# edielsonpf/speech-recognition-hmm-continuous

Measured on NVIDIA B200. Metric: frames/sec per Baum-Welch EM iteration, higher is better.
Workload: dtype f32

## Files before the change

### speech_recognition_hmm_continuous_b200/csrc/acch_kernels.cuh

```cuda
#pragma once

#include <cuda_fp16.h>

#include "dec_kernels.cuh"
#include "ws_kernels.cuh"

namespace hmmk {

constexpr int kAhSub = 64;
constexpr int kAhStages = 4;
constexpr int kAhDrain = 8;
constexpr int kAhCfWarps = kAhSub / 32;
constexpr int kAhProdWarp = 8 + kAhCfWarps;
constexpr int kAhG1Warp = kAhProdWarp + 1;
constexpr int kAhThreads = (kAhG1Warp + 2) * 32;
constexpr int kAhTmS = 256, kAhTmW = 352;
constexpr float kAhWLog2 = 14.f;

__host__ __device__ inline size_t ah_tile_bytes(int KP) { return (size_t)2 * (kAhSub / 8) * (3 * KP / 16) * 128; }
__host__ __device__ inline size_t ah_image_bytes(int KP) { return (size_t)128 * 2 * KP * 2; }
__host__ __device__ inline size_t ah_stage_bytes(int KP) { return ah_tile_bytes(KP) + kAhSub * 8 * 4; }
__host__ __device__ inline size_t ah_smem_bytes(int KP) { return kAhStages * ah_stage_bytes(KP) + 1024 + 256 + kAccImgCap * 4 + (size_t)KP * 128 * 4; }

constexpr int kAhScN = 7;
// ... 33 lines not shown
      const float *src = x32 + (int64_t)__ldg(frame_ids + tl.x + f) * DP + cc * 8;
      const float *s = sc + blk * DP + cc * 8;
      const float4 a = __ldg(reinterpret_cast<const float4 *>(src)), b = __ldg(reinterpret_cast<const float4 *>(src + 4));
      float v[8] = {a.x, a.y, a.z, a.w, b.x, b.y, b.z, b.w};
#pragma unroll
      for (int j = 0; j < 8; j++) v[j] = (blk != 1 ? v[j] * v[j] : v[j]) * s[j];
      split_half2(v[0], v[1], h.x, l.x); split_half2(v[2], v[3], h.y, l.y);
      split_half2(v[4], v[5], h.z, l.z); split_half2(v[6], v[7], h.w, l.w);
    }
    const size_t o = (size_t)fg * NCH * 128 + (size_t)c * 128 + (size_t)r * 16;
    *reinterpret_cast<uint4 *>(hi + o) = h;
    *reinterpret_cast<uint4 *>(lo + o) = l;
  }
}

__global__ void k_pack_wT_h(const double *__restrict__ mu, const double *__restrict__ iv, const float *__restrict__ kc2all,
                            const double *__restrict__ ctr, const float *__restrict__ sc, int G, int nRB, int D, int DP,
                            unsigned short *__restrict__ images, float *__restrict__ kcT) {
  const int img = blockIdx.y, v = img / nRB, rb = img - v * nRB;
  const int KP = 2 * DP;
  pdl_wait();
  unsigned short *im = images + (size_t)img * (ah_image_bytes(KP) / 2);
  for (int idx = blockIdx.x * blockDim.x + threadIdx.x; idx < 128 * KP; idx += gridDim.x * blockDim.x) {
    const int r = idx / KP, k = idx - r * KP;
    const int part = k / DP, d = k - part * DP;
    const int g = rb * 128 + r;
    float val = 0.f;
    if (g < G && d < D) {
      const int64_t gg = (int64_t)v * G + g;
      const double m = mu[gg * D + d] - ctr[d], w = iv[gg * D + d];
      val = (float)(part == 1 ? m * w * (double)sc[4 * DP + d] : -0.5 * w * (double)sc[3 * DP + d]);
    }
    unsigned short h, l;
    split_half(val, h, l);
    im[(size_t)r * 2 * KP + k] = h;
    im[(size_t)r * 2 * KP + KP + k] = l;
    if (k == 0) kcT[(size_t)img * 128 + r] = (g < G) ? kc2all[(int64_t)v * G + g] : kNegInf;
  }
}

__device__ __forceinline__ void bulk_copy_g2s(uint32_t dst_smem, const void *src, uint32_t bytes, uint32_t mbar) {
  asm volatile("cp.async.bulk.shared::cluster.global.mbarrier::complete_tx::bytes [%0], [%1], %2, [%3];" ::"r"(dst_smem), "l"(src), "r"(bytes),
               "r"(mbar)
               : "memory");
}

__global__ void __launch_bounds__(kAhThreads, 1)
k_accum_h(const TcTile *__restrict__ units, int nunits, const int32_t *__restrict__ frame_ids, const unsigned char *__restrict__ x16,
          const uint32_t *__restrict__ images, const float *__restrict__ kcT, const float *__restrict__ logb, const float *__restrict__ gamma,
          int N, int M, int G, int D, int DP, double *__restrict__ stats, int64_t stats_stride, int64_t off_S0, int64_t off_S1, int64_t off_S2,
          float *__restrict__ scratch, const float *__restrict__ dsc) {
// ... 292 lines not shown
```

### speech_recognition_hmm_continuous_b200/csrc/hmmcu.cu

```cuda
#include <cuda_runtime.h>
#include <stdarg.h>
#include <stdio.h>
#include <string.h>

#include <algorithm>
#include <atomic>
#include <map>
#include <string>
#include <utility>
#include <vector>

#include "hmm_cuda.h"
#include "kernels.cuh"
#include "fb_kernels.cuh"
#include "fbres_kernels.cuh"
#include "tc_kernels.cuh"
#include "ws_kernels.cuh"
#include "dec_kernels.cuh"
#include "acch_kernels.cuh"
#include "vit_kernels.cuh"
#include "init_kernels.cuh"

using namespace hmmk;

namespace {

char g_create_err[512] = "";
std::atomic<uint64_t> g_alloc_epoch{0};

struct DevBuf {
  void *p = nullptr;
  size_t cap = 0;
  cudaError_t ensure(size_t bytes) {
    if (bytes <= cap) return cudaSuccess;
    g_alloc_epoch++;
    if (p) cudaFree(p);
// ... 58 lines not shown
  int use_graph = 1;
  uint64_t cfg_epoch = 0;
  GraphSlot g_estep, g_mstep;
  int train_path = 0;
  std::map<std::string, Timer> timers;

  int U = 0, D = 0, DP = 0, Tmax = 0;
  int64_t F = 0;
  bool have_features = false;
  DevBuf x64_own;
  const double *d_x64 = nullptr;
  DevBuf x32, ctr, off_d, xabs_d;
  std::vector<int64_t> off;
  double kappa = 0.0;
  bool kappa_stale = true;
  DevBuf em_old, em_active, ctl_d, ext_d, upd_d;
  double *ctl_h = nullptr;
  size_t ctl_cap = 0;

  int V = 0, N = 0, M = 0, G = 0, Dm = 0;
  bool have_models = false, pack_dirty = true;
  bool banded = false;
  DevBuf A, c, mu, iv, det, mu32, iv32, k32, kc2;
  bool kc_dirty = true, simt_dirty = true;

  std::vector<int32_t> u2m;
  DevBuf u2m_d, mus_d, mu_d, tiles_d;
  DevBuf vit_map, vit_tiles;
  std::vector<int32_t> vit_u2m;
  int64_t n_vit_tiles = 0;
  uint64_t feat_epoch = 1, vit_epoch = 0;
// ... 237 lines not shown
}

void hmmcu_destroy(hmmcu_ctx *ctx) {
  if (!ctx) return;
  cudaSetDevice(ctx->dev);
  cudaStreamSynchronize(ctx->st);
  unlink_streams(ctx);
  for (void *p : ctx->peer_opened) cudaIpcCloseMemHandle(p);
  ctx->peer_area.release(); ctx->peer_ptrs_d.release(); ctx->peer_seq_d.release(); ctx->peer_stamps.release();
  ctx->logb_joint.release();
  DevBuf *bufs[] = {&ctx->x64_own, &ctx->x32, &ctx->ctr, &ctx->off_d, &ctx->A, &ctx->c, &ctx->mu, &ctx->iv, &ctx->det,
                    &ctx->mu32, &ctx->iv32, &ctx->k32, &ctx->kc2, &ctx->u2m_d, &ctx->mus_d, &ctx->mu_d, &ctx->tiles_d, &ctx->logb,
                    &ctx->post, &ctx->gamma, &ctx->alpha_ws, &ctx->stats, &ctx->logp_utt_d, &ctx->score_d,
                    &ctx->psi_ws, &ctx->path_d, &ctx->tiles_dec, &ctx->rank_in, &ctx->rank_out, &ctx->tc_train.images, &ctx->tc_train.kc, &ctx->tc_train.s0,
                    &ctx->tc_train.ns, &ctx->xabs_d, &ctx->tc_dec.images, &ctx->tc_dec.kc, &ctx->tc_dec.s0, &ctx->tc_dec.ns, &ctx->tc_tiles_train,
                    &ctx->frame_ids_d, &ctx->tc_tiles_dec, &ctx->acc_images, &ctx->acc_kc, &ctx->acc_units, &ctx->beta_ws, &ctx->acc_dbg, &ctx->em_old, &ctx->em_active, &ctx->ctl_d, &ctx->ext_d, &ctx->upd_d, &ctx->ws_train.images, &ctx->ws_train.s0, &ctx->ws_train.ns,
                    &ctx->ws_dec.images, &ctx->ws_dec.images16, &ctx->ws_dec.scales16, &ctx->ws_dec.s0, &ctx->ws_dec.ns, &ctx->ws_tiles_train, &ctx->acc_units64, &ctx->logb64, &ctx->acc_scratch, &ctx->acc_slot_start, &ctx->acc_slot_ids, &ctx->in_lst, &ctx->in_off, &ctx->in_vk, &ctx->in_cent,
                    &ctx->in_sum, &ctx->in_dist, &ctx->in_cnt, &ctx->in_idx, &ctx->in_dd, &ctx->in_ord, &ctx->vit_map, &ctx->vit_tiles,
                    &ctx->res_order, &ctx->res_upos, &ctx->res_batches, &ctx->res_counter, &ctx->ustats,
                    &ctx->acc_images16, &ctx->acc_sc, &ctx->acc_unitsH, &ctx->acc_slot_start_h, &ctx->acc_slot_ids_h, &ctx->x16, &ctx->x16_tiles};
  for (DevBuf *b : bufs) b->release();
  for (auto &kv : ctx->timers) {
    if (kv.second.a) cudaEventDestroy(kv.second.a);
    if (kv.second.b) cudaEventDestroy(kv.second.b);
    for (auto &pr : kv.second.pairs) { cudaEventDestroy(pr.first); cudaEventDestroy(pr.second); }
  }
  if (ctx->g_estep.exec) cudaGraphExecDestroy(ctx->g_estep.exec);
  if (ctx->g_mstep.exec) cudaGraphExecDestroy(ctx->g_mstep.exec);
  if (ctx->ctl_h) cudaFreeHost(ctx->ctl_h);
  if (ctx->ctr_h) cudaFreeHost(ctx->ctr_h);
  if (ctx->path_h) cudaFreeHost(ctx->path_h);
// ... 18 lines not shown
  CK(cudaSetDevice(ctx->dev));
  CK(cudaStreamSynchronize(ctx->st));
  return HMMCU_OK;
}
int hmmcu_host_alloc(void **p, uint64_t bytes) { return cudaMallocHost(p, bytes) == cudaSuccess ? HMMCU_OK : HMMCU_ENOMEM; }
void hmmcu_host_free(void *p) {
  if (p) cudaFreeHost(p);
}
int64_t hmmcu_launch_count(const hmmcu_ctx *ctx) { return ctx ? ctx->launches : 0; }
void hmmcu_enable_timing(hmmcu_ctx *ctx, int on) { ctx->timing = on != 0; ctx->cfg_epoch++; }
double hmmcu_last_kernel_ms(const hmmcu_ctx *ctx, const char *name) {
  if (strcmp(name, "kappa") == 0) return ctx->kappa;
  if (strcmp(name, "tc_active") == 0) return ctx->last_tc ? 1.0 : 0.0;
  if (strcmp(name, "dec_f16_active") == 0) return ctx->last_dec16 ? 1.0 : 0.0;
  if (strcmp(name, "acc_h_active") == 0) return ctx->last_acc_h ? 1.0 : 0.0;
  if (strcmp(name, "dec_grid") == 0) return (double)ctx->dec_grid;
  {
    const size_t ln = strlen(name);
    if (ln > 6 && strcmp(name + ln - 6, "_total") == 0) {
      auto itt = ctx->timers.find(std::string(name, ln - 6));
      if (itt == ctx->timers.end() || !itt->second.used) return -1.0;
      const Timer &t = itt->second;
      if (!t.collect) return hmmcu_last_kernel_ms(ctx, std::string(name, ln - 6).c_str());
      double tot = 0.0;
      for (size_t k = 0; k < t.npairs; k++) {
        float ms1 = 0.f;
        if (cudaEventSynchronize(t.pairs[k].second) != cudaSuccess || cudaEventElapsedTime(&ms1, t.pairs[k].first, t.pairs[k].second) != cudaSuccess) {
          cudaGetLastError();
          return -1.0;
        }
// ... 1601 lines not shown
  std::vector<int> act(V, 1);
  CK(cudaMemcpyAsync(ctx->em_old.p, one.data(), sizeof(double) * V, cudaMemcpyHostToDevice, ctx->st));
  CK(cudaMemcpyAsync(ctx->em_active.p, act.data(), sizeof(int) * V, cudaMemcpyHostToDevice, ctx->st));
  CK(cudaStreamSynchronize(ctx->st));
  return HMMCU_OK;
}

int hmmcu_mstep(hmmcu_ctx *ctx, double threshold, double *sum_logp, double *n_utt, int32_t *updated) {
  if (!ctx || !ctx->have_models || ctx->stats_n != hmmcu_stats_size(ctx->N, ctx->M, ctx->Dm) * ctx->V || !ctx->em_old.p)
    return fail(ctx, HMMCU_EINVAL, "mstep: needs hmmcu_em_reset and an E-step on the current model set");
  CK(cudaSetDevice(ctx->dev));
  const int V = ctx->V;
  int rc = ensure_ctl(ctx);
  if (rc) return rc;
  const int64_t ssz = hmmcu_stats_size(ctx->N, ctx->M, ctx->Dm);
  CK(ctx->upd_d.ensure(sizeof(int) * V));
  {
    const int DP = round_up(ctx->Dm + 1, 4);
    CK(ctx->ext_d.ensure(sizeof(unsigned long long) * (2 * DP + 1)));
  }
  const bool repack = ctx->train_path == 2 && !ctx->pack_dirty && !ctx->ws_train.dirty && !ctx->acc_dirty && !ctx->kc_dirty &&
                      ctx->have_features && ctx->Dm == ctx->D;
  auto enqueue = [&]() -> int {
    t_begin(ctx, "mstep");
    k_mstep_ctl<<<(V + 127) / 128, 128, 0, ctx->st>>>(ctx->stats.as<double>(), ssz, V, threshold, ctx->em_old.as<double>(),
                                                      ctx->em_active.as<int>(), ctx->ctl_d.as<double>(), ctx->upd_d.as<int>());
    LAUNCH_CHECK();
    CK(launch_pdl(k_mstep_apply, dim3(1 + (ctx->G + 7) / 8, V), 256, 0, ctx->st, ctx->stats.as<double>(), ssz, ctx->N, ctx->M, ctx->Dm,
                  1.0e-5 , ctx->upd_d.as<int>(), ctx->A.as<double>(), ctx->c.as<double>(),
                  ctx->mu.as<double>(), ctx->iv.as<double>(), ctx->det.as<double>()));
    LAUNCH_CHECK();
    int rc2;
    const bool fork = !ctx->timing && ctx->mstep_fork;
    auto on_stream = [&](cudaStream_t side, auto launch) -> int {
      cudaStream_t keep = ctx->st;
      ctx->st = side;
      const int r = launch();
      ctx->st = keep;
      return r;
    };
    if (fork) {
      CK(cudaEventRecord(ctx->ev_fork[0], ctx->st));
      CK(cudaStreamWaitEvent(ctx->st_aux[0], ctx->ev_fork[0], 0));
      if ((rc2 = on_stream(ctx->st_aux[0], [&] { return launch_kappa(ctx, ctx->ctl_d.as<double>() + 3 * V); })) != HMMCU_OK) return rc2;
      CK(cudaEventRecord(ctx->ev_join[0], ctx->st_aux[0]));
    } else {
      if ((rc2 = launch_kappa(ctx, ctx->ctl_d.as<double>() + 3 * V)) != HMMCU_OK) return rc2;
    }
    t_end(ctx, "mstep");
    if (repack) {
      t_begin(ctx, "pack");
      if ((rc2 = launch_pack_kc(ctx)) != HMMCU_OK) return rc2;
      if (fork) {
        CK(cudaEventRecord(ctx->ev_fork[1], ctx->st));
        CK(cudaStreamWaitEvent(ctx->st_aux[1], ctx->ev_fork[1], 0));
        if ((rc2 = on_stream(ctx->st_aux[1], [&] { return launch_pack_acc(ctx); })) != HMMCU_OK) return rc2;
        CK(cudaEventRecord(ctx->ev_join[1], ctx->st_aux[1]));
      }
      if ((rc2 = launch_pack_ws(ctx, ctx->ws_train)) != HMMCU_OK) return rc2;
      if (fork) CK(cudaStreamWaitEvent(ctx->st, ctx->ev_join[1], 0));
      else if ((rc2 = launch_pack_acc(ctx)) != HMMCU_OK) return rc2;
      t_end(ctx, "pack");
    }
    if (fork) CK(cudaStreamWaitEvent(ctx->st, ctx->ev_join[0], 0));
    CK(cudaMemcpyAsync(ctx->ctl_h, ctx->ctl_d.p, sizeof(double) * (3 * (size_t)V + 1), cudaMemcpyDeviceToHost, ctx->st));
    return HMMCU_OK;
  };
  uint64_t tbits;
  memcpy(&tbits, &threshold, sizeof(tbits));
  if ((rc = run_graphed(ctx, ctx->g_mstep, (tbits * 31u) ^ (repack ? 2u : 0u) ^ (ctx->mstep_fork ? 4u : 0u), enqueue)) != HMMCU_OK) return rc;
  CK(cudaStreamSynchronize(ctx->st));
  for (int v = 0; v < V; v++) {
    if (sum_logp) sum_logp[v] = ctx->ctl_h[v];
    if (n_utt) n_utt[v] = ctx->ctl_h[V + v];
    if (updated) updated[v] = ctx->ctl_h[2 * V + v] != 0.0;
  }
  ctx->kappa = ctx->ctl_h[3 * V];
  ctx->kappa_stale = false;
  if (repack) {
    ctx->simt_dirty = true;
    ctx->tc_train.dirty = true;
    ctx->tc_dec.dirty = true;
    ctx->ws_dec.dirty = true;
  } else {
    ctx->pack_dirty = true;
// ... 494 lines not shown
```

### speech_recognition_hmm_continuous_b200/csrc/kernels.cuh

```cuda
#pragma once
#include <cuda_runtime.h>
#include <math.h>
#include <stdint.h>

namespace hmmk {

constexpr float kNegInf = -INFINITY;
constexpr double kLogTrueMin = -744.4400719213812;

__host__ __device__ inline int round_up(int a, int b) { return (a + b - 1) / b * b; }

__device__ __forceinline__ void pdl_wait() { asm volatile("griddepcontrol.wait;" ::: "memory"); }
__device__ __forceinline__ void pdl_trigger() { asm volatile("griddepcontrol.launch_dependents;" ::: "memory"); }

__global__ void k_center(const double *__restrict__ x, int64_t F, int D, int DP, double *__restrict__ ctr) {
  __shared__ double part[16][64];
  const int d = threadIdx.x & 63, grp = threadIdx.x >> 6;
  int64_t ns = F < 4096 ? F : 4096;
  int64_t stride = F / ns;
  for (int d0 = 0; d0 < DP; d0 += 64) {
    double s = 0.0;
    if (d0 + d < D)
      for (int64_t k = grp; k < ns; k += 16) s += x[(k * stride) * D + d0 + d];
    part[grp][d] = s;
// ... 340 lines not shown
    else if (e0 < 2) sec = 1;
    else {
      int b2 = -1;
      for (int k = 0; k < e0; k++) {
        if (k == best) continue;
        if (b2 < 0 || val(k) > val(b2)) b2 = k;
      }
      sec = b2;
    }
  }
  label[u] = first;
  if (second) second[u] = sec;
}


__global__ void k_mstep_ctl(const double *__restrict__ stats, int64_t ss, int V, double threshold, double *__restrict__ em_old,
                            int *__restrict__ em_active, double *__restrict__ ctl, int *__restrict__ upd) {
  const int v = blockIdx.x * blockDim.x + threadIdx.x;
  pdl_trigger();
  if (v >= V) return;
  const double *st = stats + (int64_t)v * ss;
  const double probab = st[ss - 2], nutt = st[ss - 1];
  ctl[v] = probab;
  ctl[V + v] = nutt;
  int u = 0;
  if (em_active[v]) {
    const double variation = fabs((em_old[v] - probab) / em_old[v]);
    if (variation > threshold) { em_old[v] = probab; u = 1; }
    else em_active[v] = 0;
  }
  ctl[2 * V + v] = (double)u;
  upd[v] = u;
}

__global__ void __launch_bounds__(256)
k_mstep_apply(const double *__restrict__ stats, int64_t ss, int N, int M, int D, double floor_, const int *__restrict__ upd,
              double *__restrict__ Aall, double *__restrict__ call, double *__restrict__ muall, double *__restrict__ ivall,
              double *__restrict__ detall) {
  const int v = blockIdx.y, tid = threadIdx.x, G = N * M;
  pdl_wait();
  pdl_trigger();
  if (!upd[v]) return;
  const double *st = stats + (int64_t)v * ss;
  const double *num = st, *den = num + (int64_t)N * N, *denmix = den + N, *S0 = denmix + N;
  const double *S1 = S0 + G, *S2 = S1 + (int64_t)G * D;
  if (blockIdx.x == 0) {
    double *A = Aall + (int64_t)v * N * N, *c = call + (int64_t)v * G;
    for (int idx = tid; idx < N * N; idx += blockDim.x) {
      const int i = idx / N;
      if (den[i] != 0.0) A[idx] = num[idx] / den[i];
    }
    for (int i = tid; i < N; i += blockDim.x) {
      double *w = c + i * M;
      if (denmix[i] != 0.0)
        for (int k = 0; k < M; k++) w[k] = S0[i * M + k] / denmix[i];
      double s = 0.0;
      for (int k = 0; k < M; k++) {
        if (w[k] < floor_) w[k] = floor_;
        s += w[k];
      }
      for (int k = 0; k < M; k++) w[k] /= s;
    }
    return;
  }
  const int warp = tid >> 5, lane = tid & 31;
  const int k = (blockIdx.x - 1) * 8 + warp;
  if (k >= G) return;
  const int i = k / M;
  double *mu = muall + ((int64_t)v * G + k) * D, *iv = ivall + ((int64_t)v * G + k) * D;
  const bool fresh = denmix[i] != 0.0;
  const double s0 = S0[k];
  double dt = 1.0;
  for (int d0 = 0; d0 < D; d0 += 32) {
    const int d = d0 + lane;
    double var = 1.0;
    if (d < D) {
      if (fresh) {
        mu[d] = S1[(int64_t)k * D + d] / s0;
        var = S2[(int64_t)k * D + d] / s0;
        if (var < floor_) var = floor_;
      } else var = iv[d];
      iv[d] = 1.0 / var;
    }
    const int nd = min(32, D - d0);
    for (int j = 0; j < nd; j++) dt *= __shfl_sync(0xffffffffu, var, j);
  }
  if (lane == 0) detall[(int64_t)v * G + k] = dt;
}

__global__ void k_model_extremes(const double *__restrict__ mu, const double *__restrict__ iv, const double *__restrict__ ctr,
                                 int64_t VG, int D, int DP, unsigned long long *__restrict__ ext, const unsigned int *__restrict__ xabs,
                                 unsigned int *__restrict__ done, double *__restrict__ kappa_out) {
  const int d = threadIdx.x % DP, grp = threadIdx.x / DP, ngrp = blockDim.x / DP;
  if (d < D && grp < ngrp) {
    double ivm = 0.0, mum = 0.0;
    const double c0 = ctr[d];
    for (int64_t g = (int64_t)blockIdx.x * ngrp + grp; g < VG; g += (int64_t)gridDim.x * ngrp) {
      double a = iv[g * D + d], b = fabs(mu[g * D + d] - c0);
      if (!(a == a)) a = INFINITY;
      if (!(b == b)) b = INFINITY;
      ivm = fmax(ivm, a);
      mum = fmax(mum, b);
    }
    atomicMax(ext + d, (unsigned long long)__double_as_longlong(ivm));
    atomicMax(ext + DP + d, (unsigned long long)__double_as_longlong(mum));
  }
  __shared__ bool last;
  __threadfence();
  __syncthreads();
  if (threadIdx.x == 0) last = atomicAdd(done, 1u) == gridDim.x - 1;
  __syncthreads();
  if (!last) return;
  __threadfence();
  __shared__ double part[8];
  double t = 0.0;
  for (int dd = threadIdx.x; dd < D; dd += blockDim.x) {
    const double ivm = __longlong_as_double((long long)__ldcg(ext + dd));
    double r = __longlong_as_double((long long)__ldcg(ext + DP + dd));
    if (xabs) r = fmax(r, (double)__uint_as_float(xabs[dd]));
    const double u = 2.0 * ivm * r * r;
    t += (u == u) ? u : INFINITY;
  }
#pragma unroll
  for (int o = 16; o > 0; o >>= 1) t += __shfl_xor_sync(0xffffffffu, t, o);
  if ((threadIdx.x & 31) == 0 && (threadIdx.x >> 5) < 8) part[threadIdx.x >> 5] = t;
  __syncthreads();
  if (threadIdx.x == 0) {
    double kappa = 0.0;
    for (int w = 0; w < min(8, (int)(blockDim.x + 31) / 32); w++) kappa += part[w];
    *kappa_out = kappa;
  }
}

}
```

### speech_recognition_hmm_continuous_b200/csrc/tc_kernels.cuh

```cuda
#pragma once
#include <cuda_runtime.h>
#include <stdint.h>

#include "kernels.cuh"

namespace hmmk {

constexpr int kTcRows = 128;
constexpr int kTcThreads = 256;
constexpr int kTcMaxTN = 192;

struct TcTile {
  int32_t row0;
  int32_t nrows;
  int32_t img;
  int32_t state0;
  int32_t v;
  int32_t pad;
};

__host__ __device__ inline int tc_slab_bytes(int rows) { return rows * 32; }
__host__ __device__ inline size_t tc_image_bytes(int TN, int KP) { return (size_t)2 * (KP / 8) * tc_slab_bytes(TN); }
__host__ __device__ inline uint32_t tc_elem_off(int row, int k) {
  return (uint32_t)((row >> 3) * 256 + (((k & 7) >> 2) * 128) + ((row & 7) * 16) + ((k & 3) * 4));
// ... 330 lines not shown
__device__ __forceinline__ void tmem_wait_ld() { asm volatile("tcgen05.wait::ld.sync.aligned;" ::: "memory"); }
__device__ __forceinline__ void tmem_st16(uint32_t taddr, const uint32_t *r) {
  asm volatile(
      "tcgen05.st.sync.aligned.32x32b.x16.b32 [%0], {%1,%2,%3,%4,%5,%6,%7,%8,%9,%10,%11,%12,%13,%14,%15,%16};" ::"r"(taddr),
      "r"(r[0]), "r"(r[1]), "r"(r[2]), "r"(r[3]), "r"(r[4]), "r"(r[5]), "r"(r[6]), "r"(r[7]), "r"(r[8]), "r"(r[9]), "r"(r[10]),
      "r"(r[11]), "r"(r[12]), "r"(r[13]), "r"(r[14]), "r"(r[15])
      : "memory");
}
__device__ __forceinline__ void tmem_st8(uint32_t taddr, const uint32_t *r) {
  asm volatile("tcgen05.st.sync.aligned.32x32b.x8.b32 [%0], {%1,%2,%3,%4,%5,%6,%7,%8};" ::"r"(taddr), "r"(r[0]), "r"(r[1]), "r"(r[2]),
               "r"(r[3]), "r"(r[4]), "r"(r[5]), "r"(r[6]), "r"(r[7])
               : "memory");
}
__device__ __forceinline__ void tmem_wait_st() { asm volatile("tcgen05.wait::st.sync.aligned;" ::: "memory"); }

__global__ void k_pack_kc(const double *__restrict__ mu, const double *__restrict__ iv, const double *__restrict__ det,
                          const double *__restrict__ c, const double *__restrict__ ctr, int64_t VG, int D, float *__restrict__ kc2) {
  const int64_t g = ((int64_t)blockIdx.x * blockDim.x + threadIdx.x) >> 5;
  const int lane = threadIdx.x & 31;
  pdl_wait();
  pdl_trigger();
  if (g >= VG) return;
  double q = 0.0;
  for (int d = lane; d < D; d += 32) {
    const double m = mu[g * D + d] - ctr[d];
    q += m * m * iv[g * D + d];
  }
#pragma unroll
  for (int o = 16; o > 0; o >>= 1) q += __shfl_xor_sync(0xffffffffu, q, o);
  if (lane == 0) {
    double k = -INFINITY;
    const double dt = det[g], cc = c[g];
    if (dt != 0.0 && cc > 0.0) k = (log(cc) - 0.5 * ((double)D * 1.8378770664093453 + log(fabs(dt))) - 0.5 * q) * 1.4426950408889634;
    kc2[g] = (float)k;
  }
}

__global__ void k_pack_wT_tc(const double *__restrict__ mu, const double *__restrict__ iv, const float *__restrict__ kc2all,
                             const double *__restrict__ ctr, int G, int nRB, int D, int DP, float *__restrict__ images,
                             float *__restrict__ kcT) {
  const int img = blockIdx.y, v = img / nRB, rb = img - v * nRB;
  const int KP = 2 * DP;
  float *im = images + (size_t)img * (tc_accT_image_bytes(KP) / 4);
  for (int idx = blockIdx.x * blockDim.x + threadIdx.x; idx < 128 * KP; idx += gridDim.x * blockDim.x) {
    const int r = idx / KP, k = idx - r * KP;
    const int part = k / DP, d = k - part * DP;
    const int g = rb * 128 + r;
    float val = 0.f;
    if (g < G && d < D) {
      const int64_t gg = (int64_t)v * G + g;
      const double m = mu[gg * D + d] - ctr[d], w = iv[gg * D + d];
      val = (float)(part == 0 ? m * w : -0.5 * w);
    }
    float h, l;
    split_tf32(val, h, l);
    im[(size_t)r * 2 * KP + k] = h;
    im[(size_t)r * 2 * KP + KP + k] = l;
    if (k == 0) kcT[(size_t)img * 128 + r] = (g < G) ? kc2all[(int64_t)v * G + g] : kNegInf;
  }
}

__global__ void __launch_bounds__(kTcThreads, 1)
k_accum_tc(const TcTile *__restrict__ units, int nunits, const int32_t *__restrict__ frame_ids, const float *__restrict__ x32,
           const float *__restrict__ images, const float *__restrict__ kcT, const float *__restrict__ logb,
           const float *__restrict__ gamma, int N, int M, int G, int D, int DP, double *__restrict__ stats,
           int64_t stats_stride, int64_t off_S0, int64_t off_S1, int64_t off_S2, float *__restrict__ dbg) {
  extern __shared__ __align__(1024) uint8_t smem_raw[];
  __shared__ uint64_t mbar;
  __shared__ uint32_t tmem_base_s;
  const int KP = 2 * DP, KP2 = tc_kp2(KP), NSLAB = KP / 8;
  const uint32_t PX = (uint32_t)(KP / 4) * 128;
  uint8_t *sm = (uint8_t *)(((uintptr_t)smem_raw + 1023) & ~(uintptr_t)1023);
// ... 227 lines not shown
```

### speech_recognition_hmm_continuous_b200/csrc/ws_kernels.cuh

```cuda
#pragma once
#include <cuda_fp16.h>
#include "tc_kernels.cuh"

namespace hmmk {

constexpr int kWsEpiWarps = 8;
constexpr int kWsThreads = (kWsEpiWarps + 9) * 32;
constexpr int kWsMaxTN = 96;
constexpr int kWsMaxTN1 = 176;
constexpr int kWsXch = 6;

__host__ __device__ inline size_t ws_image_bytes(int TN, int KP) { return (size_t)2 * (TN / 8) * (KP / 4) * 128 + (size_t)TN * 4; }
__host__ __device__ inline size_t ws_emis_smem_bytes(int TN, int KP) { return ws_image_bytes(TN, KP) + 1024 + 272; }

__host__ __device__ inline int ws_pad_m(int M) {
  if (M > 16) return (M + 15) / 16 * 16;
  if (M == 3 || M == 5) return M;
  int p = 1;
  while (p < M) p <<= 1;
  return p;
}
__host__ __device__ inline int ws_states_per_chunk(int MPd) { return MPd <= 16 ? 16 / MPd : 1; }
__host__ __device__ inline int ws_image_cols(int MPd, int nstates) {
  if (MPd > 16) return nstates * MPd;
// ... 57 lines not shown
  float4 v;
  asm volatile("ld.shared.v4.f32 {%0, %1, %2, %3}, [%4];" : "=f"(v.x), "=f"(v.y), "=f"(v.z), "=f"(v.w) : "r"(addr));
  return v;
}
__device__ __forceinline__ float lds_f32(uint32_t addr) {
  float v;
  asm volatile("ld.shared.f32 %0, [%1];" : "=f"(v) : "r"(addr));
  return v;
}
__device__ __forceinline__ int lds_i32(uint32_t addr) {
  int v;
  asm volatile("ld.shared.s32 %0, [%1];" : "=r"(v) : "r"(addr));
  return v;
}
__device__ __forceinline__ void sts_f32(uint32_t addr, float v) { asm volatile("st.shared.f32 [%0], %1;" ::"r"(addr), "f"(v) : "memory"); }

__global__ void k_pack_w_ws(const double *__restrict__ mu, const double *__restrict__ iv, const float *__restrict__ kc2all,
                            const double *__restrict__ ctr, int M, int MP, int D, int DP, int TN,
                            const int32_t *__restrict__ img_state0, const int32_t *__restrict__ img_nstates,
                            float *__restrict__ images) {
  const int img = blockIdx.y;
  const int KP = 2 * DP;
  pdl_wait();
  const uint32_t P = (uint32_t)(KP / 4) * 128;
  const size_t img_floats = ws_image_bytes(TN, KP) / 4;
  float *hi = images + (size_t)img * img_floats;
  float *lo = hi + (size_t)(TN / 8) * (P / 4);
  float *kc2 = lo + (size_t)(TN / 8) * (P / 4);
  const int64_t s0g = img_state0[img];
  const int nst = img_nstates[img];
  auto gauss_of = [&](int n) -> int64_t {
    int st, m;
    if (MP > 16) { st = n / MP; m = n - st * MP; }
    else {
      const int spc = 16 / MP, c = n >> 4, w = n & 15;
      if (w >= spc * MP) return -1;
      st = c * spc + w / MP; m = w % MP;
    }
    return (st < nst && m < M) ? (s0g + st) * M + m : -1;
  };
  for (int idx = blockIdx.x * blockDim.x + threadIdx.x; idx < TN * KP; idx += gridDim.x * blockDim.x) {
    const int n = idx / KP, k = idx - n * KP;
    const int part = k / DP, d = k - part * DP;
    const int64_t g = gauss_of(n);
    float val = 0.f;
    if (g >= 0 && d < D) {
      const double m = mu[g * D + d] - ctr[d], w = iv[g * D + d];
      val = (float)(part == 0 ? m * w : -0.5 * w);
    }
    float h, l;
    split_tf32(val, h, l);
    const size_t o = ((size_t)(n & 7) * 16 + (k & 3) * 4 + (size_t)(k >> 2) * 128 + (size_t)(n >> 3) * P) / 4;
    hi[o] = h;
    lo[o] = l;
    if (k == 0) kc2[n] = (g >= 0) ? kc2all[g] : kNegInf;
  }
}

__host__ __device__ inline size_t dec16_image_bytes(int TN, int KP) { return (size_t)2 * (TN / 8) * (KP / 8) * 128 + (size_t)TN * 4; }

__global__ void k_dec16_scales(const unsigned long long *__restrict__ ext, const unsigned int *__restrict__ xabs, int D, int DP, float *__restrict__ sc) {
  const int d = threadIdx.x;
  if (d >= DP) return;
  float s1 = 1.f, s2 = 1.f;
  bool dead = false;
  if (d < D) {
    const double ivm = __longlong_as_double((long long)ext[d]), mum = __longlong_as_double((long long)ext[DP + d]);
    const double r = xabs ? (double)__uint_as_float(xabs[d]) : mum;
    const double wl = mum * ivm;
// ... 903 lines not shown
```

Baseline: 1.801 billion.

## Fuse M-step control, update, kappa, and weight repacking into one kernel

Replaces the M-step pipeline with a single kernel launched one CTA per (state, model). The old pipeline was a control kernel, an apply kernel, a kappa/extremes kernel on a forked stream and three pack kernels. The new kernel updates A, mixture weights, means, variances and determinants, and writes the tensor-core weight images and kc2 constants in place. A last-block reduction then computes the per-dimension extremes, kappa and the control flags. This removes several launches, a stream fork and join, and re-reading mu/iv for packing. In exchange it relies on a grid-wide last-block pattern with atomics and a persistent scratch buffer, and it drops the device-to-host copy of the control array, which is now written directly to a host pointer.

Result: faster. 1.978 billion (median of 6 runs) (+9.8%).

```diff
diff --git a/speech_recognition_hmm_continuous_b200/csrc/acch_kernels.cuh b/speech_recognition_hmm_continuous_b200/csrc/acch_kernels.cuh
--- a/speech_recognition_hmm_continuous_b200/csrc/acch_kernels.cuh
+++ b/speech_recognition_hmm_continuous_b200/csrc/acch_kernels.cuh
@@ -71,6 +71,16 @@
   }
 }
 
+__device__ __forceinline__ float w_h_val(double mu, double iv, double ctr, const float *sc, int DP, int d, int part) {
+  const double m = mu - ctr;
+  return (float)(part == 1 ? m * iv * (double)sc[4 * DP + d] : -0.5 * iv * (double)sc[3 * DP + d]);
+}
+__device__ __forceinline__ void acc_h_put(unsigned short *im, int KP, int r, int k, float val) {
+  unsigned short h, l;
+  split_half(val, h, l);
+  im[(size_t)r * 2 * KP + k] = h;
+  im[(size_t)r * 2 * KP + KP + k] = l;
+}
 __global__ void k_pack_wT_h(const double *__restrict__ mu, const double *__restrict__ iv, const float *__restrict__ kc2all,
                             const double *__restrict__ ctr, const float *__restrict__ sc, int G, int nRB, int D, int DP,
                             unsigned short *__restrict__ images, float *__restrict__ kcT) {
@@ -85,13 +95,9 @@
     float val = 0.f;
     if (g < G && d < D) {
       const int64_t gg = (int64_t)v * G + g;
-      const double m = mu[gg * D + d] - ctr[d], w = iv[gg * D + d];
-      val = (float)(part == 1 ? m * w * (double)sc[4 * DP + d] : -0.5 * w * (double)sc[3 * DP + d]);
-    }
-    unsigned short h, l;
-    split_half(val, h, l);
-    im[(size_t)r * 2 * KP + k] = h;
-    im[(size_t)r * 2 * KP + KP + k] = l;
+      val = w_h_val(mu[gg * D + d], iv[gg * D + d], ctr[d], sc, DP, d, part);
+    }
+    acc_h_put(im, KP, r, k, val);
     if (k == 0) kcT[(size_t)img * 128 + r] = (g < G) ? kc2all[(int64_t)v * G + g] : kNegInf;
   }
 }
diff --git a/speech_recognition_hmm_continuous_b200/csrc/hmmcu.cu b/speech_recognition_hmm_continuous_b200/csrc/hmmcu.cu
--- a/speech_recognition_hmm_continuous_b200/csrc/hmmcu.cu
+++ b/speech_recognition_hmm_continuous_b200/csrc/hmmcu.cu
@@ -20,6 +20,7 @@
 #include "acch_kernels.cuh"
 #include "vit_kernels.cuh"
 #include "init_kernels.cuh"
+#include "mstep_kernels.cuh"
 
 using namespace hmmk;
 
@@ -108,7 +109,8 @@
   std::vector<int64_t> off;
   double kappa = 0.0;
   bool kappa_stale = true;
-  DevBuf em_old, em_active, ctl_d, ext_d, upd_d;
+  DevBuf em_old, em_active, ctl_d, ext_d;
+  DevBuf mstep_scr;
   double *ctl_h = nullptr;
   size_t ctl_cap = 0;
 
@@ -376,7 +378,7 @@
                     &ctx->post, &ctx->gamma, &ctx->alpha_ws, &ctx->stats, &ctx->logp_utt_d, &ctx->score_d,
                     &ctx->psi_ws, &ctx->path_d, &ctx->tiles_dec, &ctx->rank_in, &ctx->rank_out, &ctx->tc_train.images, &ctx->tc_train.kc, &ctx->tc_train.s0,
                     &ctx->tc_train.ns, &ctx->xabs_d, &ctx->tc_dec.images, &ctx->tc_dec.kc, &ctx->tc_dec.s0, &ctx->tc_dec.ns, &ctx->tc_tiles_train,
-                    &ctx->frame_ids_d, &ctx->tc_tiles_dec, &ctx->acc_images, &ctx->acc_kc, &ctx->acc_units, &ctx->beta_ws, &ctx->acc_dbg, &ctx->em_old, &ctx->em_active, &ctx->ctl_d, &ctx->ext_d, &ctx->upd_d, &ctx->ws_train.images, &ctx->ws_train.s0, &ctx->ws_train.ns,
+                    &ctx->frame_ids_d, &ctx->tc_tiles_dec, &ctx->acc_images, &ctx->acc_kc, &ctx->acc_units, &ctx->beta_ws, &ctx->acc_dbg, &ctx->em_old, &ctx->em_active, &ctx->ctl_d, &ctx->ext_d, &ctx->mstep_scr, &ctx->ws_train.images, &ctx->ws_train.s0, &ctx->ws_train.ns,
                     &ctx->ws_dec.images, &ctx->ws_dec.images16, &ctx->ws_dec.scales16, &ctx->ws_dec.s0, &ctx->ws_dec.ns, &ctx->ws_tiles_train, &ctx->acc_units64, &ctx->logb64, &ctx->acc_scratch, &ctx->acc_slot_start, &ctx->acc_slot_ids, &ctx->in_lst, &ctx->in_off, &ctx->in_vk, &ctx->in_cent,
                     &ctx->in_sum, &ctx->in_dist, &ctx->in_cnt, &ctx->in_idx, &ctx->in_dd, &ctx->in_ord, &ctx->vit_map, &ctx->vit_tiles,
                     &ctx->res_order, &ctx->res_upos, &ctx->res_batches, &ctx->res_counter, &ctx->ustats,
@@ -425,6 +427,7 @@
   if (strcmp(name, "tc_active") == 0) return ctx->last_tc ? 1.0 : 0.0;
   if (strcmp(name, "dec_f16_active") == 0) return ctx->last_dec16 ? 1.0 : 0.0;
   if (strcmp(name, "acc_h_active") == 0) return ctx->last_acc_h ? 1.0 : 0.0;
+  if (strcmp(name, "train_path") == 0) return (double)ctx->train_path;
   if (strcmp(name, "dec_grid") == 0) return (double)ctx->dec_grid;
   {
     const size_t ln = strlen(name);
@@ -2056,61 +2059,52 @@
   int rc = ensure_ctl(ctx);
   if (rc) return rc;
   const int64_t ssz = hmmcu_stats_size(ctx->N, ctx->M, ctx->Dm);
-  CK(ctx->upd_d.ensure(sizeof(int) * V));
+  const int N = ctx->N, M = ctx->M, D = ctx->Dm, DP = round_up(D + 1, 4);
+  CK(ctx->ext_d.ensure(sizeof(unsigned long long) * (2 * DP + 1)));
   {
-    const int DP = round_up(ctx->Dm + 1, 4);
-    CK(ctx->ext_d.ensure(sizeof(unsigned long long) * (2 * DP + 1)));
+    const size_t cap0 = ctx->mstep_scr.cap;
+    CK(ctx->mstep_scr.ensure(sizeof(unsigned long long) * (2 * DP + 1)));
+    if (ctx->mstep_scr.cap != cap0) CK(cudaMemsetAsync(ctx->mstep_scr.p, 0, ctx->mstep_scr.cap, ctx->st));
   }
   const bool repack = ctx->train_path == 2 && !ctx->pack_dirty && !ctx->ws_train.dirty && !ctx->acc_dirty && !ctx->kc_dirty &&
                       ctx->have_features && ctx->Dm == ctx->D;
+  MstepPack pk = {};
+  if (repack) {
+    hmmcu_ctx::TcSet &ts = ctx->ws_train;
+    pk.kc2 = ctx->kc2.as<float>();
+    pk.ws = ts.images.as<float>();
+    pk.ws_TN = ts.TN;
+    pk.ws_SCt = ts.SCt;
+    pk.ws_ipw = (N + ts.SCt - 1) / ts.SCt;
+    pk.ws_MP = ws_pad_m(M);
+    if (h_acc_on(ctx)) {
+      pk.acc_h = ctx->acc_images16.as<unsigned short>();
+      pk.acc_sc = ctx->acc_sc.as<float>();
+    } else {
+      pk.acc_tc = ctx->acc_images.as<float>();
+    }
+    pk.acc_kc = ctx->acc_kc.as<float>();
+    pk.nRB = (ctx->G + 127) / 128;
+  }
+  const int threads = 32 * std::min(std::max(M, 8), 16);
+  const size_t smem = sizeof(double) * (M + 2 * (size_t)DP);
+  if (smem > 227 * 1024) return fail(ctx, HMMCU_EINVAL, "mstep: M=%d, D=%d do not fit one CTA's shared memory", M, D);
+  if (smem > 48 * 1024) CK(cudaFuncSetAttribute(k_mstep, cudaFuncAttributeMaxDynamicSharedMemorySize, (int)smem));
   auto enqueue = [&]() -> int {
     t_begin(ctx, "mstep");
-    k_mstep_ctl<<<(V + 127) / 128, 128, 0, ctx->st>>>(ctx->stats.as<double>(), ssz, V, threshold, ctx->em_old.as<double>(),
-                                                      ctx->em_active.as<int>(), ctx->ctl_d.as<double>(), ctx->upd_d.as<int>());
+    k_mstep<<<dim3(N, V), threads, smem, ctx->st>>>(ctx->stats.as<double>(), ssz, V, N, M, D, DP, 1.0e-5 ,
+                                                     threshold, ctx->em_old.as<double>(), ctx->em_active.as<int>(), ctx->A.as<double>(),
+                                                     ctx->c.as<double>(), ctx->mu.as<double>(), ctx->iv.as<double>(), ctx->det.as<double>(),
+                                                     ctx->ctr.as<double>(), pk, ctx->mstep_scr.as<unsigned long long>(),
+                                                     ctx->ext_d.as<unsigned long long>(), ctx->F > 0 ? ctx->xabs_d.as<unsigned int>() : nullptr,
+                                                     ctx->ctl_h);
     LAUNCH_CHECK();
-    CK(launch_pdl(k_mstep_apply, dim3(1 + (ctx->G + 7) / 8, V), 256, 0, ctx->st, ctx->stats.as<double>(), ssz, ctx->N, ctx->M, ctx->Dm,
-                  1.0e-5 , ctx->upd_d.as<int>(), ctx->A.as<double>(), ctx->c.as<double>(),
-                  ctx->mu.as<double>(), ctx->iv.as<double>(), ctx->det.as<double>()));
-    LAUNCH_CHECK();
-    int rc2;
-    const bool fork = !ctx->timing && ctx->mstep_fork;
-    auto on_stream = [&](cudaStream_t side, auto launch) -> int {
-      cudaStream_t keep = ctx->st;
-      ctx->st = side;
-      const int r = launch();
-      ctx->st = keep;
-      return r;
-    };
-    if (fork) {
-      CK(cudaEventRecord(ctx->ev_fork[0], ctx->st));
-      CK(cudaStreamWaitEvent(ctx->st_aux[0], ctx->ev_fork[0], 0));
-      if ((rc2 = on_stream(ctx->st_aux[0], [&] { return launch_kappa(ctx, ctx->ctl_d.as<double>() + 3 * V); })) != HMMCU_OK) return rc2;
-      CK(cudaEventRecord(ctx->ev_join[0], ctx->st_aux[0]));
-    } else {
-      if ((rc2 = launch_kappa(ctx, ctx->ctl_d.as<double>() + 3 * V)) != HMMCU_OK) return rc2;
-    }
     t_end(ctx, "mstep");
-    if (repack) {
-      t_begin(ctx, "pack");
-      if ((rc2 = launch_pack_kc(ctx)) != HMMCU_OK) return rc2;
-      if (fork) {
-        CK(cudaEventRecord(ctx->ev_fork[1], ctx->st));
-        CK(cudaStreamWaitEvent(ctx->st_aux[1], ctx->ev_fork[1], 0));
-        if ((rc2 = on_stream(ctx->st_aux[1], [&] { return launch_pack_acc(ctx); })) != HMMCU_OK) return rc2;
-        CK(cudaEventRecord(ctx->ev_join[1], ctx->st_aux[1]));
-      }
-      if ((rc2 = launch_pack_ws(ctx, ctx->ws_train)) != HMMCU_OK) return rc2;
-      if (fork) CK(cudaStreamWaitEvent(ctx->st, ctx->ev_join[1], 0));
-      else if ((rc2 = launch_pack_acc(ctx)) != HMMCU_OK) return rc2;
-      t_end(ctx, "pack");
-    }
-    if (fork) CK(cudaStreamWaitEvent(ctx->st, ctx->ev_join[0], 0));
-    CK(cudaMemcpyAsync(ctx->ctl_h, ctx->ctl_d.p, sizeof(double) * (3 * (size_t)V + 1), cudaMemcpyDeviceToHost, ctx->st));
     return HMMCU_OK;
   };
   uint64_t tbits;
   memcpy(&tbits, &threshold, sizeof(tbits));
-  if ((rc = run_graphed(ctx, ctx->g_mstep, (tbits * 31u) ^ (repack ? 2u : 0u) ^ (ctx->mstep_fork ? 4u : 0u), enqueue)) != HMMCU_OK) return rc;
+  if ((rc = run_graphed(ctx, ctx->g_mstep, (tbits * 31u) ^ (repack ? 2u : 0u), enqueue)) != HMMCU_OK) return rc;
   CK(cudaStreamSynchronize(ctx->st));
   for (int v = 0; v < V; v++) {
     if (sum_logp) sum_logp[v] = ctx->ctl_h[v];
diff --git a/speech_recognition_hmm_continuous_b200/csrc/kernels.cuh b/speech_recognition_hmm_continuous_b200/csrc/kernels.cuh
--- a/speech_recognition_hmm_continuous_b200/csrc/kernels.cuh
+++ b/speech_recognition_hmm_continuous_b200/csrc/kernels.cuh
@@ -378,78 +378,28 @@
 }
 
 
-__global__ void k_mstep_ctl(const double *__restrict__ stats, int64_t ss, int V, double threshold, double *__restrict__ em_old,
-                            int *__restrict__ em_active, double *__restrict__ ctl, int *__restrict__ upd) {
-  const int v = blockIdx.x * blockDim.x + threadIdx.x;
-  pdl_trigger();
-  if (v >= V) return;
-  const double *st = stats + (int64_t)v * ss;
-  const double probab = st[ss - 2], nutt = st[ss - 1];
-  ctl[v] = probab;
-  ctl[V + v] = nutt;
-  int u = 0;
-  if (em_active[v]) {
-    const double variation = fabs((em_old[v] - probab) / em_old[v]);
-    if (variation > threshold) { em_old[v] = probab; u = 1; }
-    else em_active[v] = 0;
-  }
-  ctl[2 * V + v] = (double)u;
-  upd[v] = u;
-}
-
-__global__ void __launch_bounds__(256)
-k_mstep_apply(const double *__restrict__ stats, int64_t ss, int N, int M, int D, double floor_, const int *__restrict__ upd,
-              double *__restrict__ Aall, double *__restrict__ call, double *__restrict__ muall, double *__restrict__ ivall,
-              double *__restrict__ detall) {
-  const int v = blockIdx.y, tid = threadIdx.x, G = N * M;
-  pdl_wait();
-  pdl_trigger();
-  if (!upd[v]) return;
-  const double *st = stats + (int64_t)v * ss;
-  const double *num = st, *den = num + (int64_t)N * N, *denmix = den + N, *S0 = denmix + N;
-  const double *S1 = S0 + G, *S2 = S1 + (int64_t)G * D;
-  if (blockIdx.x == 0) {
-    double *A = Aall + (int64_t)v * N * N, *c = call + (int64_t)v * G;
-    for (int idx = tid; idx < N * N; idx += blockDim.x) {
-      const int i = idx / N;
-      if (den[i] != 0.0) A[idx] = num[idx] / den[i];
-    }
-    for (int i = tid; i < N; i += blockDim.x) {
-      double *w = c + i * M;
-      if (denmix[i] != 0.0)
-        for (int k = 0; k < M; k++) w[k] = S0[i * M + k] / denmix[i];
-      double s = 0.0;
-      for (int k = 0; k < M; k++) {
-        if (w[k] < floor_) w[k] = floor_;
-        s += w[k];
-      }
-      for (int k = 0; k < M; k++) w[k] /= s;
-    }
-    return;
-  }
-  const int warp = tid >> 5, lane = tid & 31;
-  const int k = (blockIdx.x - 1) * 8 + warp;
-  if (k >= G) return;
-  const int i = k / M;
-  double *mu = muall + ((int64_t)v * G + k) * D, *iv = ivall + ((int64_t)v * G + k) * D;
-  const bool fresh = denmix[i] != 0.0;
-  const double s0 = S0[k];
-  double dt = 1.0;
-  for (int d0 = 0; d0 < D; d0 += 32) {
-    const int d = d0 + lane;
-    double var = 1.0;
-    if (d < D) {
-      if (fresh) {
-        mu[d] = S1[(int64_t)k * D + d] / s0;
-        var = S2[(int64_t)k * D + d] / s0;
-        if (var < floor_) var = floor_;
-      } else var = iv[d];
-      iv[d] = 1.0 / var;
-    }
-    const int nd = min(32, D - d0);
-    for (int j = 0; j < nd; j++) dt *= __shfl_sync(0xffffffffu, var, j);
-  }
-  if (lane == 0) detall[(int64_t)v * G + k] = dt;
+__device__ __forceinline__ void extremes_kappa(const unsigned long long *ext, const unsigned int *xabs, int D, int DP, double *kappa_out) {
+  __shared__ double part[8];
+  const int tid = threadIdx.x;
+  if (tid < 256) {
+    double t = 0.0;
+    for (int dd = tid; dd < D; dd += 256) {
+      const double ivm = __longlong_as_double((long long)__ldcg(ext + dd));
+      double r = __longlong_as_double((long long)__ldcg(ext + DP + dd));
+      if (xabs) r = fmax(r, (double)__uint_as_float(xabs[dd]));
+      const double u = 2.0 * ivm * r * r;
+      t += (u == u) ? u : INFINITY;
+    }
+#pragma unroll
+    for (int o = 16; o > 0; o >>= 1) t += __shfl_xor_sync(0xffffffffu, t, o);
+    if ((tid & 31) == 0) part[tid >> 5] = t;
+  }
+  __syncthreads();
+  if (tid == 0) {
+    double kappa = 0.0;
+    for (int w = 0; w < 8; w++) kappa += part[w];
+    *kappa_out = kappa;
+  }
 }
 
 __global__ void k_model_extremes(const double *__restrict__ mu, const double *__restrict__ iv, const double *__restrict__ ctr,
@@ -476,24 +426,7 @@
   __syncthreads();
   if (!last) return;
   __threadfence();
-  __shared__ double part[8];
-  double t = 0.0;
-  for (int dd = threadIdx.x; dd < D; dd += blockDim.x) {
-    const double ivm = __longlong_as_double((long long)__ldcg(ext + dd));
-    double r = __longlong_as_double((long long)__ldcg(ext + DP + dd));
-    if (xabs) r = fmax(r, (double)__uint_as_float(xabs[dd]));
-    const double u = 2.0 * ivm * r * r;
-    t += (u == u) ? u : INFINITY;
-  }
-#pragma unroll
-  for (int o = 16; o > 0; o >>= 1) t += __shfl_xor_sync(0xffffffffu, t, o);
-  if ((threadIdx.x & 31) == 0 && (threadIdx.x >> 5) < 8) part[threadIdx.x >> 5] = t;
-  __syncthreads();
-  if (threadIdx.x == 0) {
-    double kappa = 0.0;
-    for (int w = 0; w < min(8, (int)(blockDim.x + 31) / 32); w++) kappa += part[w];
-    *kappa_out = kappa;
-  }
-}
-
-}
+  extremes_kappa(ext, xabs, D, DP, kappa_out);
+}
+
+}
diff --git a/speech_recognition_hmm_continuous_b200/csrc/mstep_kernels.cuh b/speech_recognition_hmm_continuous_b200/csrc/mstep_kernels.cuh
--- /dev/null
+++ b/speech_recognition_hmm_continuous_b200/csrc/mstep_kernels.cuh
@@ -0,0 +1,186 @@
+#pragma once
+
+#include "acch_kernels.cuh"
+
+namespace hmmk {
+
+__device__ __forceinline__ int mstep_rule(double probab, double old, int active, double threshold) {
+  if (!active) return 0;
+  const double variation = fabs((old - probab) / old);
+  return variation > threshold ? 1 : 0;
+}
+
+struct MstepPack {
+  float *kc2;
+  float *ws;
+  int ws_TN, ws_SCt, ws_ipw, ws_MP;
+  float *acc_tc;
+  unsigned short *acc_h;
+  const float *acc_sc;
+  float *acc_kc;
+  int nRB;
+};
+
+__global__ void __launch_bounds__(512)
+k_mstep(const double *__restrict__ stats, int64_t ss, int V, int N, int M, int D, int DP, double floor_, double threshold,
+        double *__restrict__ em_old, int *__restrict__ em_active, double *__restrict__ Aall, double *__restrict__ call,
+        double *__restrict__ muall, double *__restrict__ ivall, double *__restrict__ detall, const double *__restrict__ ctr,
+        MstepPack pk, unsigned long long *__restrict__ scr, unsigned long long *__restrict__ ext,
+        const unsigned int *__restrict__ xabs, double *__restrict__ ctl) {
+  extern __shared__ double sm_w[];
+  unsigned long long *sx = reinterpret_cast<unsigned long long *>(sm_w + M);
+  __shared__ double s_sum;
+  __shared__ bool last;
+  const int i = blockIdx.x, v = blockIdx.y, tid = threadIdx.x, warp = tid >> 5, lane = tid & 31, nw = blockDim.x >> 5;
+  const int G = N * M, KP = 2 * DP;
+  for (int t = tid; t < 2 * DP; t += blockDim.x) sx[t] = 0ull;
+
+  const double *st = stats + (int64_t)v * ss;
+  const int u = mstep_rule(st[ss - 2], em_old[v], em_active[v], threshold);
+  const double *num = st, *den = num + (int64_t)N * N, *denmix = den + N, *S0 = denmix + N;
+  const double *S1 = S0 + G, *S2 = S1 + (int64_t)G * D;
+  const bool fresh = u && denmix[i] != 0.0;
+
+  double *cst = call + (int64_t)v * G + (int64_t)i * M;
+  if (u) {
+    if (den[i] != 0.0)
+      for (int j = tid; j < N; j += blockDim.x) Aall[(int64_t)v * N * N + i * N + j] = num[i * N + j] / den[i];
+    for (int m = tid; m < M; m += blockDim.x) {
+      double w = fresh ? S0[i * M + m] / denmix[i] : cst[m];
+      if (w < floor_) w = floor_;
+      sm_w[m] = w;
+    }
+  }
+  __syncthreads();
+  if (u && tid == 0) {
+    double s = 0.0;
+    for (int m = 0; m < M; m++) s += sm_w[m];
+    s_sum = s;
+  }
+  __syncthreads();
+  if (u)
+    for (int m = tid; m < M; m += blockDim.x) {
+      const double w = sm_w[m] / s_sum;
+      sm_w[m] = w;
+      cst[m] = w;
+    }
+  __syncthreads();
+
+  const bool pack = u && pk.ws != nullptr;
+  const uint32_t P = (uint32_t)(KP / 4) * 128;
+  float *ws_hi = nullptr, *ws_lo = nullptr, *ws_kc = nullptr;
+  double ivm0 = 0.0, mum0 = 0.0, ivm1 = 0.0, mum1 = 0.0;
+  if (pack) {
+    ws_hi = pk.ws + (size_t)(v * pk.ws_ipw + i / pk.ws_SCt) * (ws_image_bytes(pk.ws_TN, KP) / 4);
+    ws_lo = ws_hi + (size_t)(pk.ws_TN / 8) * (P / 4);
+    ws_kc = ws_lo + (size_t)(pk.ws_TN / 8) * (P / 4);
+  }
+  for (int m = warp; m < M; m += nw) {
+    const int gi = i * M + m;
+    const int64_t g = (int64_t)v * G + gi;
+    double *mu = muall + g * D, *iv = ivall + g * D;
+    const double s0 = fresh ? S0[gi] : 1.0;
+    const int n = pack ? ws_row_of(i % pk.ws_SCt, m, pk.ws_MP) : 0;
+    const int aimg = v * pk.nRB + gi / 128, ar = gi % 128;
+    double dt = 1.0, q = 0.0;
+    for (int d0 = 0; d0 < D; d0 += 32) {
+      const int d = d0 + lane;
+      double var = 1.0;
+      if (d < D) {
+        double mud, ivd;
+        const double cd = ctr[d];
+        if (u) {
+          if (fresh) {
+            mud = S1[(int64_t)gi * D + d] / s0;
+            mu[d] = mud;
+            var = S2[(int64_t)gi * D + d] / s0;
+            if (var < floor_) var = floor_;
+          } else {
+            mud = mu[d];
+            var = iv[d];
+          }
+          ivd = 1.0 / var;
+          iv[d] = ivd;
+        } else {
+          mud = mu[d];
+          ivd = iv[d];
+        }
+        if (pack) {
+          q = kc_term(q, mud, ivd, cd);
+          for (int part = 0; part < 2; part++) {
+            const int k = part * DP + d;
+            ws_put(ws_hi, ws_lo, P, n, k, w_tf32_val(mud, ivd, cd, part));
+            if (pk.acc_h)
+              acc_h_put(pk.acc_h + (size_t)aimg * (ah_image_bytes(KP) / 2), KP, ar, k, w_h_val(mud, ivd, cd, pk.acc_sc, DP, d, part));
+            else
+              acc_tc_put(pk.acc_tc + (size_t)aimg * (tc_accT_image_bytes(KP) / 4), KP, ar, k, w_tf32_val(mud, ivd, cd, part));
+          }
+        }
+        double a = ivd, b = fabs(mud - cd);
+        if (!(a == a)) a = INFINITY;
+        if (!(b == b)) b = INFINITY;
+        if (d0 == 0) {
+          ivm0 = fmax(ivm0, a);
+          mum0 = fmax(mum0, b);
+        } else if (d0 == 32) {
+          ivm1 = fmax(ivm1, a);
+          mum1 = fmax(mum1, b);
+        } else {
+          atomicMax(sx + d, (unsigned long long)__double_as_longlong(fmax(0.0, a)));
+          atomicMax(sx + DP + d, (unsigned long long)__double_as_longlong(fmax(0.0, b)));
+        }
+      }
+      if (u) {
+        const int nd = min(32, D - d0);
+        for (int j = 0; j < nd; j++) dt *= __shfl_sync(0xffffffffu, var, j);
+      }
+    }
+    if (u && lane == 0) detall[g] = dt;
+    if (pack) {
+      const float k2 = kc2_of(q, dt, sm_w[m], D);
+      if (lane == 0) {
+        pk.kc2[g] = k2;
+        ws_kc[n] = k2;
+        pk.acc_kc[(size_t)aimg * 128 + ar] = k2;
+      }
+    }
+  }
+  if (lane < D) {
+    atomicMax(sx + lane, (unsigned long long)__double_as_longlong(ivm0));
+    atomicMax(sx + DP + lane, (unsigned long long)__double_as_longlong(mum0));
+  }
+  if (lane + 32 < D) {
+    atomicMax(sx + 32 + lane, (unsigned long long)__double_as_longlong(ivm1));
+    atomicMax(sx + DP + 32 + lane, (unsigned long long)__double_as_longlong(mum1));
+  }
+  __syncthreads();
+  for (int t = tid; t < 2 * DP; t += blockDim.x)
+    if (sx[t]) atomicMax(scr + t, sx[t]);
+
+  unsigned int *done = reinterpret_cast<unsigned int *>(scr + 2 * DP);
+  __threadfence();
+  __syncthreads();
+  if (tid == 0) last = atomicAdd(done, 1u) == gridDim.x * gridDim.y - 1;
+  __syncthreads();
+  if (!last) return;
+  __threadfence();
+  for (int w = tid; w < V; w += blockDim.x) {
+    const double *sw = stats + (int64_t)w * ss;
+    const double probab = sw[ss - 2];
+    const int uw = mstep_rule(probab, em_old[w], em_active[w], threshold);
+    if (uw) em_old[w] = probab;
+    else if (em_active[w]) em_active[w] = 0;
+    ctl[w] = probab;
+    ctl[V + w] = sw[ss - 1];
+    ctl[2 * V + w] = (double)uw;
+  }
+  extremes_kappa(scr, xabs, D, DP, ctl + 3 * V);
+  __syncthreads();
+  for (int t = tid; t < 2 * DP; t += blockDim.x) {
+    ext[t] = __ldcg(scr + t);
+    scr[t] = 0ull;
+  }
+  if (tid == 0) *done = 0u;
+}
+
+}
diff --git a/speech_recognition_hmm_continuous_b200/csrc/tc_kernels.cuh b/speech_recognition_hmm_continuous_b200/csrc/tc_kernels.cuh
--- a/speech_recognition_hmm_continuous_b200/csrc/tc_kernels.cuh
+++ b/speech_recognition_hmm_continuous_b200/csrc/tc_kernels.cuh
@@ -368,6 +368,18 @@
 }
 __device__ __forceinline__ void tmem_wait_st() { asm volatile("tcgen05.wait::st.sync.aligned;" ::: "memory"); }
 
+__device__ __forceinline__ double kc_term(double q, double mu, double iv, double ctr) {
+  const double m = mu - ctr;
+  return q + m * m * iv;
+}
+__device__ __forceinline__ float kc2_of(double q, double dt, double cc, int D) {
+#pragma unroll
+  for (int o = 16; o > 0; o >>= 1) q += __shfl_xor_sync(0xffffffffu, q, o);
+  double k = -INFINITY;
+  if (dt != 0.0 && cc > 0.0) k = (log(cc) - 0.5 * ((double)D * 1.8378770664093453 + log(fabs(dt))) - 0.5 * q) * 1.4426950408889634;
+  return (float)k;
+}
+
 __global__ void k_pack_kc(const double *__restrict__ mu, const double *__restrict__ iv, const double *__restrict__ det,
                           const double *__restrict__ c, const double *__restrict__ ctr, int64_t VG, int D, float *__restrict__ kc2) {
   const int64_t g = ((int64_t)blockIdx.x * blockDim.x + threadIdx.x) >> 5;
@@ -376,18 +388,20 @@
   pdl_trigger();
   if (g >= VG) return;
   double q = 0.0;
-  for (int d = lane; d < D; d += 32) {
-    const double m = mu[g * D + d] - ctr[d];
-    q += m * m * iv[g * D + d];
-  }
-#pragma unroll
-  for (int o = 16; o > 0; o >>= 1) q += __shfl_xor_sync(0xffffffffu, q, o);
-  if (lane == 0) {
-    double k = -INFINITY;
-    const double dt = det[g], cc = c[g];
-    if (dt != 0.0 && cc > 0.0) k = (log(cc) - 0.5 * ((double)D * 1.8378770664093453 + log(fabs(dt))) - 0.5 * q) * 1.4426950408889634;
-    kc2[g] = (float)k;
-  }
+  for (int d = lane; d < D; d += 32) q = kc_term(q, mu[g * D + d], iv[g * D + d], ctr[d]);
+  const float k = kc2_of(q, det[g], c[g], D);
+  if (lane == 0) kc2[g] = k;
+}
+
+__device__ __forceinline__ float w_tf32_val(double mu, double iv, double ctr, int part) {
+  const double m = mu - ctr;
+  return (float)(part == 0 ? m * iv : -0.5 * iv);
+}
+__device__ __forceinline__ void acc_tc_put(float *im, int KP, int r, int k, float val) {
+  float h, l;
+  split_tf32(val, h, l);
+  im[(size_t)r * 2 * KP + k] = h;
+  im[(size_t)r * 2 * KP + KP + k] = l;
 }
 
 __global__ void k_pack_wT_tc(const double *__restrict__ mu, const double *__restrict__ iv, const float *__restrict__ kc2all,
@@ -403,13 +417,9 @@
     float val = 0.f;
     if (g < G && d < D) {
       const int64_t gg = (int64_t)v * G + g;
-      const double m = mu[gg * D + d] - ctr[d], w = iv[gg * D + d];
-      val = (float)(part == 0 ? m * w : -0.5 * w);
-    }
-    float h, l;
-    split_tf32(val, h, l);
-    im[(size_t)r * 2 * KP + k] = h;
-    im[(size_t)r * 2 * KP + KP + k] = l;
+      val = w_tf32_val(mu[gg * D + d], iv[gg * D + d], ctr[d], part);
+    }
+    acc_tc_put(im, KP, r, k, val);
     if (k == 0) kcT[(size_t)img * 128 + r] = (g < G) ? kc2all[(int64_t)v * G + g] : kNegInf;
   }
 }
diff --git a/speech_recognition_hmm_continuous_b200/csrc/ws_kernels.cuh b/speech_recognition_hmm_continuous_b200/csrc/ws_kernels.cuh
--- a/speech_recognition_hmm_continuous_b200/csrc/ws_kernels.cuh
+++ b/speech_recognition_hmm_continuous_b200/csrc/ws_kernels.cuh
@@ -95,6 +95,19 @@
   return v;
 }
 __device__ __forceinline__ void sts_f32(uint32_t addr, float v) { asm volatile("st.shared.f32 [%0], %1;" ::"r"(addr), "f"(v) : "memory"); }
+
+__device__ __forceinline__ int ws_row_of(int st, int m, int MP) {
+  if (MP > 16) return st * MP + m;
+  const int spc = 16 / MP;
+  return (st / spc) * 16 + (st % spc) * MP + m;
+}
+__device__ __forceinline__ void ws_put(float *hi, float *lo, uint32_t P, int n, int k, float val) {
+  float h, l;
+  split_tf32(val, h, l);
+  const size_t o = ((size_t)(n & 7) * 16 + (k & 3) * 4 + (size_t)(k >> 2) * 128 + (size_t)(n >> 3) * P) / 4;
+  hi[o] = h;
+  lo[o] = l;
+}
 
 __global__ void k_pack_w_ws(const double *__restrict__ mu, const double *__restrict__ iv, const float *__restrict__ kc2all,
                             const double *__restrict__ ctr, int M, int MP, int D, int DP, int TN,
@@ -125,15 +138,8 @@
     const int part = k / DP, d = k - part * DP;
     const int64_t g = gauss_of(n);
     float val = 0.f;
-    if (g >= 0 && d < D) {
-      const double m = mu[g * D + d] - ctr[d], w = iv[g * D + d];
-      val = (float)(part == 0 ? m * w : -0.5 * w);
-    }
-    float h, l;
-    split_tf32(val, h, l);
-    const size_t o = ((size_t)(n & 7) * 16 + (k & 3) * 4 + (size_t)(k >> 2) * 128 + (size_t)(n >> 3) * P) / 4;
-    hi[o] = h;
-    lo[o] = l;
+    if (g >= 0 && d < D) val = w_tf32_val(mu[g * D + d], iv[g * D + d], ctr[d], part);
+    ws_put(hi, lo, P, n, k, val);
     if (k == 0) kc2[n] = (g >= 0) ? kc2all[g] : kNegInf;
   }
 }
```
